# lh3/minimap2

Hardware: AMD Instinct MI355X
Metric: aligned Gbases/sec (map-ont, 10 kb reads, -a) (higher is better)
Workload: dtype int8 (ksw2 difference DP) / int32+f32 (chaining)

## Files before the change

include/mm2amd.h:

```cpp
#ifndef MM2AMD_H
#define MM2AMD_H

#include <stdint.h>
#include <stddef.h>

#ifdef __cplusplus
extern "C" {
#endif

#define MM2AMD_EINVAL  (-1)
#define MM2AMD_ENODEV  (-2)
#define MM2AMD_EHIP    (-3)
#define MM2AMD_ENOMEM  (-4)
#define MM2AMD_ESTATE  (-5)
#define MM2AMD_EIO     (-6)

const char *mm2amd_last_error(void);
int mm2amd_last_error_code(void);
int mm2amd_version(void);
int mm2amd_host_cpus(void);
int mm2amd_device_count(void);


typedef struct {
// ... 23 lines not shown
#define MM2AMD_FIN_MAX_OPS 7168
typedef struct {
	const uint8_t *query, *target;
	int32_t qlen, tlen;
	int32_t n_pieces;
	const uint32_t *const *piece;
	const int32_t *piece_len;
} mm2amd_fin_job_t;
typedef struct { int32_t n_cigar, blen, mlen, n_ambi, dp_max, qshift, tshift, is_spliced; uint32_t cigar_off; } mm2amd_fin_res_t;
int mm2amd_update_extra_batch(int n_jobs, const mm2amd_fin_job_t *jobs, const int8_t *mat25, int8_t q, int8_t e, int log_gap,
                              mm2amd_fin_res_t *res, uint32_t *cigar_pool, size_t cigar_pool_cap);

#define MM2AMD_TXT_CIGAR   0
#define MM2AMD_TXT_CS      1
#define MM2AMD_TXT_CS_LONG 2
#define MM2AMD_TXT_MD      3
typedef struct { const uint8_t *query, *target; int32_t qlen, tlen; const uint32_t *cigar; int32_t n_cigar; } mm2amd_txt_job_t;
typedef struct { uint64_t off; uint32_t len; int32_t status; } mm2amd_txt_res_t;
int mm2amd_aln_text_batch(int n_jobs, const mm2amd_txt_job_t *jobs, int what, mm2amd_txt_res_t *res, char *pool, size_t pool_cap);

#define MM2AMD_LL_QREV  1
#define MM2AMD_LL_QCOMP 2
#define MM2AMD_LL_TREV  4
#define MM2AMD_LL_PATH_WAVE 0
#define MM2AMD_LL_PATH_WG   1
#define MM2AMD_LL_PATH_HOST 2
typedef struct { const uint8_t *query, *target; int32_t qlen, tlen; int32_t flag; } mm2amd_ll_job_t;
typedef struct { int32_t score, qe, te, path; } mm2amd_ll_res_t;
int mm2amd_ksw_ll_batch(int n_jobs, const mm2amd_ll_job_t *jobs, int8_t m, const int8_t *mat, int gapo, int gape, mm2amd_ll_res_t *res);
int mm2amd_ksw_ll_limits(int *strip_cols, int *wg_waves, int64_t *wg_min_cells, int *max_len);

int mm2amd_sort_pairs_u64(uint64_t *keys, uint64_t *vals, uint64_t n, int bits);
int mm2amd_exclusive_sum_u32(const uint32_t *in, uint32_t *out, uint64_t n);

int mm2amd_ksw_extz2_batch(int n_jobs, const mm2amd_ksw_job_t *jobs, int8_t m, const int8_t *mat, int8_t gapo, int8_t gape,
                           mm2amd_ksw_res_t *res, uint32_t *cigar_pool, size_t cigar_pool_cap);

int mm2amd_ksw_exts2_batch(int n_jobs, const mm2amd_ksw_job_t *jobs, int8_t m, const int8_t *mat, int8_t gapo, int8_t gape, int8_t gapo2, int8_t noncan,
                           mm2amd_ksw_res_t *res, uint32_t *cigar_pool, size_t cigar_pool_cap);

#ifdef MINIMAP2_H
typedef mm_idx_t mm2amd_idx_t; typedef mm_mapopt_t mm2amd_mapopt_t; typedef mm_reg1_t mm2amd_reg1_t;
struct mm2amd_bseq1_s;
#define MM2AMD_BSEQ_PTR const void *
#define MM2AMD_REG_PP   void **
#else
typedef void mm2amd_idx_t; typedef void mm2amd_mapopt_t;
#define MM2AMD_BSEQ_PTR const void *
#define MM2AMD_REG_PP   void **
#endif

void mm2amd_idxopt_init(void *io);
void mm2amd_mapopt_init(void *mo);
int mm2amd_set_opt(const char *preset, void *io, void *mo);
int mm2amd_check_opt(const void *io, const void *mo);

typedef struct mm2amd_index_s mm2amd_index_t;
mm2amd_index_t *mm2amd_idx_str(int w, int k, int is_hpc, int bucket_bits, int n, const char **seq, const char **name);
void mm2amd_idx_destroy(mm2amd_index_t *idx);
int mm2amd_idx_stat(const mm2amd_index_t *idx, int *k, int *w, int *flag, uint32_t *n_seq, uint64_t *sum_len,
                    uint64_t *n_distinct, uint64_t *n_minimizers);
int32_t mm2amd_idx_cal_max_occ(const mm2amd_index_t *idx, float f);
int mm2amd_mapopt_update(void *mo, const mm2amd_index_t *idx);
int mm2amd_idx_table_shape(const mm2amd_index_t *idx, int *bucket_bits, int *key_shift);
int mm2amd_idx_export(const mm2amd_index_t *idx, uint32_t *bucket_start, uint64_t *keys, uint32_t *val_off, uint64_t *pos, uint32_t *S);

// ... 64 lines not shown
```

minimap2_amd/__init__.py:

```python
import ctypes as C
import os

_HERE = os.path.dirname(os.path.abspath(__file__))
LIB_PATH = os.path.join(_HERE, "libmm2amd.so")


class Mm2AmdError(RuntimeError):
    pass


class KswJob(C.Structure):
    _fields_ = [("query", C.c_void_p), ("target", C.c_void_p), ("qlen", C.c_int32), ("tlen", C.c_int32), ("w", C.c_int32),
                ("zdrop", C.c_int32), ("end_bonus", C.c_int32), ("flag", C.c_int32)]


class FinJob(C.Structure):
    _fields_ = [("query", C.c_void_p), ("target", C.c_void_p), ("qlen", C.c_int32), ("tlen", C.c_int32), ("n_pieces", C.c_int32),
                ("piece", C.POINTER(C.POINTER(C.c_uint32))), ("piece_len", C.POINTER(C.c_int32))]


class FinRes(C.Structure):
    _fields_ = [("n_cigar", C.c_int32), ("blen", C.c_int32), ("mlen", C.c_int32), ("n_ambi", C.c_int32), ("dp_max", C.c_int32), ("qshift", C.c_int32),
                ("tshift", C.c_int32), ("is_spliced", C.c_int32), ("cigar_off", C.c_uint32)]

# ... 94 lines not shown
    L.mm_gpu_map_staged.argtypes = [ip, C.POINTER(vp), ip, ip]
    L.mm_gpu_batch_stage_queued.argtypes = [C.c_int, ip, ip, vp]
    L.mm_gpu_batch_discard.restype = None
    L.mm2amd_free_regs.argtypes = [C.c_int, ip, C.POINTER(vp)]
    L.mm2amd_free_regs.restype = None
    L.mm2amd_last_stats.argtypes = [C.POINTER(C.c_double), C.c_int]
    L.mm2amd_pack_regs.argtypes = [C.c_int, ip, C.POINTER(vp), vp, C.c_int64]
    L.mm2amd_pack_regs.restype = C.c_int64
    L.mm2amd_unpack_regs.argtypes = [vp, C.c_int64, C.c_int, ip, C.POINTER(vp)]
    L.mm_gpu_init_multi.argtypes = [vp, vp, C.c_int, C.c_int, ip]
    L.mm_gpu_context_generation.restype = C.c_uint64
    L.mm_gpu_destroy_if.argtypes = [C.c_uint64]
    if hasattr(L, "mm2amd_idx_str"):
        L.mm2amd_ksw_extd2_batch.restype = C.c_int
        L.mm2amd_ksw_extd2_batch.argtypes = [C.c_int, C.POINTER(KswJob), C.c_int8, C.c_char_p, C.c_int8, C.c_int8, C.c_int8,
                                             C.c_int8, C.POINTER(KswRes), C.POINTER(C.c_uint32), C.c_size_t]
        L.mm2amd_ksw_extz2_batch.restype = C.c_int
        L.mm2amd_ksw_extz2_batch.argtypes = [C.c_int, C.POINTER(KswJob), C.c_int8, C.c_char_p, C.c_int8, C.c_int8, C.POINTER(KswRes),
                                             C.POINTER(C.c_uint32), C.c_size_t]
        L.mm2amd_ksw_exts2_batch.restype = C.c_int
        L.mm2amd_ksw_exts2_batch.argtypes = [C.c_int, C.POINTER(KswJob), C.c_int8, C.c_char_p, C.c_int8, C.c_int8, C.c_int8, C.c_int8,
                                             C.POINTER(KswRes), C.POINTER(C.c_uint32), C.c_size_t]
        L.mm2amd_update_extra_batch.restype = C.c_int
        L.mm2amd_update_extra_batch.argtypes = [C.c_int, C.POINTER(FinJob), C.c_char_p, C.c_int8, C.c_int8, C.c_int, C.POINTER(FinRes), C.POINTER(C.c_uint32), C.c_size_t]
        L.mm2amd_aln_text_batch.argtypes = [C.c_int, C.POINTER(TxtJob), C.c_int, C.POINTER(TxtRes), vp, C.c_size_t]
        L.mm2amd_hits_text_batch.argtypes = [vp, C.c_int, C.POINTER(vp), C.POINTER(C.c_char_p), C.POINTER(C.c_int32), C.c_int, C.c_int, C.POINTER(TxtRes), vp,
                                             C.c_size_t]
        L.mm2amd_idx_getseq.argtypes = [vp, C.c_uint32, C.c_uint32, C.c_uint32, vp]
        if hasattr(L, "mm2amd_ksw_ll_batch"):
            L.mm2amd_ksw_ll_batch.argtypes = [C.c_int, C.POINTER(LlJob), C.c_int8, C.c_char_p, C.c_int, C.c_int, C.POINTER(LlRes)]
            L.mm2amd_ksw_ll_limits.argtypes = [ip, ip, C.POINTER(C.c_int64), ip]
        L.mm2amd_sort_pairs_u64.argtypes = [vp, vp, C.c_uint64, C.c_int]
        L.mm2amd_exclusive_sum_u32.argtypes = [vp, vp, C.c_uint64]
        L.mm2amd_idx_str.restype = vp
        L.mm2amd_idx_str.argtypes = [C.c_int, C.c_int, C.c_int, C.c_int, C.c_int, C.POINTER(C.c_char_p), C.POINTER(C.c_char_p)]
        L.mm2amd_idx_destroy.argtypes = [vp]
        L.mm2amd_idx_destroy.restype = None
        L.mm2amd_idx_stat.argtypes = [vp, ip, ip, ip, C.POINTER(C.c_uint32), C.POINTER(C.c_uint64), C.POINTER(C.c_uint64),
                                      C.POINTER(C.c_uint64)]
        L.mm2amd_idx_cal_max_occ.argtypes = [vp, C.c_float]
        L.mm2amd_idx_cal_max_occ.restype = C.c_int32
        L.mm2amd_mapopt_update.argtypes = [vp, vp]
        L.mm2amd_idx_table_shape.argtypes = [vp, ip, ip]
        L.mm2amd_idx_export.argtypes = [vp, vp, vp, vp, vp, vp]
        L.mm2amd_idx_dump.argtypes = [vp, C.c_char_p, C.c_int, C.c_int]
        L.mm2amd_idx_load.restype = vp
        L.mm2amd_idx_load.argtypes = [C.c_char_p, C.c_int, ip]
        L.mm2amd_idx_is_idx.argtypes = [C.c_char_p]
        L.mm2amd_idx_seq.argtypes = [vp, C.c_uint32, C.POINTER(C.c_char_p), C.POINTER(C.c_uint32)]
        L.mm2amd_idx_io_stats.argtypes = [C.POINTER(C.c_double), C.c_int]
        L.mm_gpu_init_index.argtypes = [vp, vp, C.c_int]
        L.mm_gpu_init_index_multi.argtypes = [vp, vp, C.c_int, C.c_int, ip]
        L.mm2amd_set_opt.argtypes = [C.c_char_p, vp, vp]
        L.mm2amd_check_opt.argtypes = [vp, vp]
        L.mm2amd_idxopt_init.argtypes = [vp]
        L.mm2amd_mapopt_init.argtypes = [vp]
        L.mm_gpu_format_batch.argtypes = [C.c_int, ip, ip, vp, ip, C.POINTER(vp), ip, C.POINTER(C.c_void_p), C.POINTER(C.c_size_t)]
        L.mm_gpu_format_batch_view.argtypes = [C.c_int, ip, ip, vp, ip, C.POINTER(vp), ip, C.POINTER(C.c_void_p), C.POINTER(C.c_size_t)]
        L.mm_gpu_format_batch_dev.argtypes = [C.c_int, ip, ip, vp, ip, C.POINTER(vp), ip, C.POINTER(C.c_void_p), C.POINTER(C.c_size_t), ip]
        L.mm2amd_profile_enable.argtypes = [C.c_int]
        L.mm2amd_profile_enable.restype = None
        L.mm2amd_profile_get.argtypes = [C.POINTER(KernelStat), C.c_int]
    return L


def host_cpus():
# ... 156 lines not shown
    _check(lib().mm2amd_ksw_ll_batch(n, arr, 5, bytes(mat), gapo, gape, res))
    return [(r.score, r.qe, r.te, r.path) for r in res[:n]]


def ksw_ll_limits():
    a, b, d, c = C.c_int(0), C.c_int(0), C.c_int(0), C.c_int64(0)
    _check(lib().mm2amd_ksw_ll_limits(C.byref(a), C.byref(b), C.byref(c), C.byref(d)))
    return {"strip_cols": a.value, "wg_waves": b.value, "wg_min_cells": c.value, "max_len": d.value}


def hits_text(idx, hits, reads, what, is_qstrand=False):
    n = len(hits)
    harr = (C.c_void_p * max(n, 1))(*hits)
    rb = [r.encode() if isinstance(r, str) else bytes(r) for r in reads]
    qarr, qlen = (C.c_char_p * max(n, 1))(*rb), (C.c_int32 * max(n, 1))(*[len(r) for r in rb])
    L = lib()
    return _texts(lambda res, pool, cap: L.mm2amd_hits_text_batch(idx, n, harr, qarr, qlen, what, 1 if is_qstrand else 0, res, pool, cap), n)


def sort_pairs_u64(keys, vals, bits=64):
    import numpy as np
    k, v = np.ascontiguousarray(keys, dtype=np.uint64).copy(), np.ascontiguousarray(vals, dtype=np.uint64).copy()
    assert k.shape == v.shape and k.ndim == 1
    _check(lib().mm2amd_sort_pairs_u64(k.ctypes.data, v.ctypes.data, k.size, bits))
    return k, v


def exclusive_sum_u32(a):
    import numpy as np
    x = np.ascontiguousarray(a, dtype=np.uint32)
    out = np.empty(x.size + 1, dtype=np.uint32)
    _check(lib().mm2amd_exclusive_sum_u32(x.ctypes.data, out.ctypes.data, x.size))
    return out


def ksw_extz2_batch(jobs, mat, gapo, gape):
    return ksw_extd2_batch(jobs, mat, gapo, gape, None, None)


def ksw_exts2_batch(jobs, mat, gapo, gape, gapo2, noncan):
    return ksw_extd2_batch(jobs, mat, gapo, gape, gapo2, None, noncan=noncan)


def ksw_extd2_batch(jobs, mat, gapo, gape, gapo2, gape2, noncan=None):
    n = len(jobs)
    arr = (KswJob * n)()
    keep = []
    tot = 0
    for i, (q, t, w, zdrop, end_bonus, flag) in enumerate(jobs):
        qb, tb = bytes(q), bytes(t)
        keep.append((qb, tb))
        arr[i].query = C.cast(C.c_char_p(qb), C.c_void_p)
        arr[i].target = C.cast(C.c_char_p(tb), C.c_void_p)
        arr[i].qlen, arr[i].tlen, arr[i].w, arr[i].zdrop, arr[i].end_bonus, arr[i].flag = len(qb), len(tb), w, zdrop, end_bonus, flag
        tot += len(qb) + len(tb)
    res = (KswRes * n)()
    pool = (C.c_uint32 * max(tot, 1))()
    if noncan is not None:
        _check(lib().mm2amd_ksw_exts2_batch(n, arr, 5, bytes(mat), gapo, gape, gapo2, noncan, res, pool, max(tot, 1)))
    elif gapo2 is None:
        _check(lib().mm2amd_ksw_extz2_batch(n, arr, 5, bytes(mat), gapo, gape, res, pool, max(tot, 1)))
    else:
        _check(lib().mm2amd_ksw_extd2_batch(n, arr, 5, bytes(mat), gapo, gape, gapo2, gape2, res, pool, max(tot, 1)))
    out = []
    for r in res:
        out.append((r.max, r.zdropped, r.max_q, r.max_t, r.mqe, r.mqe_t, r.mte, r.mte_q, r.score, r.reach_end,
# ... 384 lines not shown
```

minimap2_amd/csrc/backend_hip.cpp:

```cpp
#include <atomic>
#include <condition_variable>
#include <algorithm>
#include <cstdio>
#include <cstring>
#include <memory>
#include <mutex>
#include <numeric>
#include <stdexcept>
#include <thread>
#include "backend.hpp"
#include "chain_dump.hpp"
#include "chain_host.hpp"
#include "device_ctx.hpp"
#include "ksw_host.hpp"
#include "seed_chain_dev.hpp"
#include "index_build.hpp"
#include "kernel_prof.hpp"
#include "threads.hpp"
#include "trace.hpp"
#include "sdust_core.hpp"

namespace mm2amd {

extern const uint8_t kNt4Table[256];
// ... 289 lines not shown
		B.sort_key_in = ln.d_skey_in.p, B.sort_val_in = ln.d_sval_in.p, B.sort_key_out = ln.d_skey_out.p, B.sort_val_out = ln.d_sval_out.p, B.tie_flag = ln.d_tie.p;
		B.tie_list = ln.d_tie.p + n, B.tie_count = ln.d_tie.p + 2 * n;
		B.rid_bits = rid_bits_;
		int n_class[kAnchorSortClasses] = { 0 }, class_first[kAnchorSortClasses + 1] = { 0 };
		double a_class[kAnchorSortClasses] = { 0 };
		for (size_t i = 0; i < n; ++i) if (h_na[i]) { const int c = anchor_sort_class(h_na[i], rid_bits_); ++n_class[c], a_class[c] += h_na[i]; }
		for (int c = 0; c < kAnchorSortClasses; ++c) class_first[c + 1] = class_first[c] + n_class[c];
		uint32_t *h_list = ln.h_sort_list.ensure(n + 1);
		{
			int fill[kAnchorSortClasses];
			for (int c = 0; c < kAnchorSortClasses; ++c) fill[c] = class_first[c];
			for (size_t i = 0; i < n; ++i) if (h_na[i]) h_list[fill[anchor_sort_class(h_na[i], rid_bits_)]++] = (uint32_t)i;
		}
		ln.d_sort_list.ensure(n + 1);
		if (class_first[kAnchorSortClasses]) HIP_CHECK(hipMemcpyAsync(ln.d_sort_list.p, h_list, (size_t)class_first[kAnchorSortClasses] * 4, hipMemcpyHostToDevice, st));
		B.a_off = ln.d_a_off.p, B.mp_off = ln.d_mp_off.p, B.anchors = ln.d_anchors.p, B.mini_pos = ln.d_minipos.p;
		B.f = ln.d_f.p, B.p = ln.d_p.p, B.t = ln.d_t.p;
		kp.begin(st); launch_seed_expand(B, I_, P, st); kp.end(st, "seed_expand_kernel", 24.0 * n_a);
		launch_anchor_sort(B, I_, P, ln.d_sort_list.p, n_class, a_class, st, &kp);
		if (getenv("MM2AMD_TIE_COUNT")) {
			std::vector<uint32_t> tf(n);
			stream_wait(st);
			HIP_CHECK(hipMemcpy(tf.data(), ln.d_tie.p, n * 4, hipMemcpyDeviceToHost));
			size_t n_tied = 0;
			for (size_t i = 0; i < n; ++i) n_tied += tf[i] != 0;
			fprintf(stderr, "[mm2amd] anchor sort: %zu of %zu reads have duplicated keys (%d / %d / %d reads in the 7 k / 10 k / global classes)\n", n_tied, n, n_class[3], n_class[4], n_class[5]);
		}
		if (const char *dump = getenv("MM2AMD_SEED_DUMP")) {
			std::vector<Anchor> all(n_a + 1);
			stream_wait(st);
			if (n_a) HIP_CHECK(hipMemcpy(all.data(), ln.d_anchors.p, n_a * sizeof(Anchor), hipMemcpyDeviceToHost));
			static std::mutex dump_mu;
			std::lock_guard<std::mutex> lk(dump_mu);
			if (FILE *fp = fopen(dump, "a")) {
				for (size_t i = 0; i < n; ++i) {
					fprintf(fp, "QR\t%s\t%d\nRS\t%d\n", read_names_.empty() || !read_names_[lo + i] ? "*" : read_names_[lo + i], P.mid_occ, h_rep[i]);
					for (uint64_t j = a_off[i]; j < a_off[i + 1]; ++j) {
						const Anchor &a = all[j];
						fprintf(fp, "SD\t%s\t%d\t%c\t%d\t%d\t%d\n", (*fi_names_)[a.x << 1 >> 33].c_str(), (int32_t)a.x, "+-"[a.x >> 63], (int32_t)a.y, (int32_t)(a.y >> 32 & 0xff),
						        j == a_off[i] ? 0 : ((int32_t)a.y - (int32_t)all[j - 1].y) - ((int32_t)a.x - (int32_t)all[j - 1].x));
					}
				}
				fclose(fp);
			}
		}
		const char *cdump = P.chain_dump ? chain_dump_path() : nullptr;
		auto dump_block = [&](size_t i) {
			ChainDumpBlock b;
			b.name = read_names_.empty() ? nullptr : read_names_[lo + i];
			b.qlen = (int)(seq_off_[lo + i + 1] - seq_off_[lo + i]), b.n_seg = has_pairs_ ? unit_first_[lo + i + 1] - unit_first_[lo + i] : 1;
			return b;
		};
		if (P.anchors_only) {
			Anchor *ha = ln.h_anchors.ensure(n_a + 1);
			uint64_t *hmp = ln.h_minipos.ensure(n_mp + 1);
			if (n_a) HIP_CHECK(hipMemcpyAsync(ha, ln.d_anchors.p, n_a * sizeof(Anchor), hipMemcpyDeviceToHost, st));
			if (n_mp) HIP_CHECK(hipMemcpyAsync(hmp, ln.d_minipos.p, n_mp * 8, hipMemcpyDeviceToHost, st));
			stream_wait(st);
			Trace::get().add(lane_id, "gpu:expand+sort, d2h:anchors", tt, Trace::now());
			kp.collect();
			if (cdump) {
				std::string txt;
				for (size_t i = 0; i < n; ++i) {
					ChainDumpBlock b = dump_block(i);
					b.handed_back = true, b.in = ha + a_off[i], b.n_in = (int64_t)(a_off[i + 1] - a_off[i]);
					chain_dump_format(txt, P, b);
				}
				chain_dump_flush(cdump, txt);
			}
			parallel_for(n_threads, (long)n, [&](long i, int) {
				ReadChains &c = out[i];
				c.rep_len = h_rep[i];
				c.mp_p = hmp + mp_off[i], c.n_mp = (int32_t)(mp_off[i + 1] - mp_off[i]);
// ... 626 lines not shown
```

minimap2_amd/csrc/capi_kernels.cpp:

```cpp
#include <mutex>
#include <string>
#include <vector>
#include <cstring>
#include "../../include/mm2amd.h"
#include "hip_util.hpp"
#include "device_ctx.hpp"
#include "ksw_host.hpp"
#include "kernel_prof.hpp"
#include "region_finish.hpp"
#include "aln_text.hpp"
#include "ksw_ll.hpp"
#include "device_sort.hpp"
#include <map>

namespace mm2amd { int capi_fail(int code, const std::string &msg); }
using namespace mm2amd;

namespace {

int fail(int code, const std::string &msg) { return capi_fail(code, msg); }

struct KernelApiState {
	KswRunner ksw;
	DevBuf<uint8_t> d_qpool, d_tpool;
};
KernelApiState &kstate() { static KernelApiState s; return s; }

struct LlApiState {
	DevBuf<uint8_t> d_q, d_t;
	DevBuf<LlJob> d_jobs;
	DevBuf<LlRes> d_res;
	DevBuf<uint32_t> d_bnd;
	PinBuf<uint8_t> h_q, h_t;
	PinBuf<LlJob> h_jobs;
	PinBuf<LlRes> h_res;
};
LlApiState &ll_state() { static LlApiState s; return s; }
constexpr size_t kLlBndBudget = (size_t)1 << 26;

bool ll_no_wg() { const char *e = getenv("MM2AMD_LL_NO_WG"); return e && *e && strcmp(e, "0") != 0; }
int64_t ll_wg_min_cells() { const char *e = getenv("MM2AMD_LL_WG_MIN_CELLS"); return e && *e ? (int64_t)strtoll(e, nullptr, 10) : kLlWgMinCells; }

template <typename F>
int guarded(F &&f)
{
// ... 370 lines not shown
	return guarded([&]() -> int {
		DeviceCtx &dc = device_ctx();
		std::lock_guard<std::mutex> lk(dc.mu);
		ensure_device(dc);
		DevBuf<uint64_t> k0, v0, k1, v1;
		k0.ensure(n, 1.0), v0.ensure(n, 1.0), k1.ensure(n, 1.0), v1.ensure(n, 1.0);
		HIP_CHECK(hipMemcpyAsync(k0.p, keys, n * 8, hipMemcpyHostToDevice, dc.stream));
		HIP_CHECK(hipMemcpyAsync(v0.p, vals, n * 8, hipMemcpyHostToDevice, dc.stream));
		const int where = device_sort_pairs_u64(k0.p, v0.p, k1.p, v1.p, n, bits, dc.stream);
		HIP_CHECK(hipMemcpyAsync(keys, where ? k1.p : k0.p, n * 8, hipMemcpyDeviceToHost, dc.stream));
		HIP_CHECK(hipMemcpyAsync(vals, where ? v1.p : v0.p, n * 8, hipMemcpyDeviceToHost, dc.stream));
		HIP_CHECK(hipStreamSynchronize(dc.stream));
		return 0;
	});
}

int mm2amd_exclusive_sum_u32(const uint32_t *in, uint32_t *out, uint64_t n)
{
	if (!out || (n > 0 && !in) || n >= (1ull << 32)) return fail(MM2AMD_EINVAL, "[mm2amd] exclusive_sum_u32: bad arguments (n < 2^32)");
	return guarded([&]() -> int {
		DeviceCtx &dc = device_ctx();
		std::lock_guard<std::mutex> lk(dc.mu);
		ensure_device(dc);
		DevBuf<uint32_t> d;
		d.ensure(n + 1, 1.0);
		if (n) HIP_CHECK(hipMemcpyAsync(d.p, in, n * 4, hipMemcpyHostToDevice, dc.stream));
		device_exclusive_sum_u32(d.p, d.p, n, dc.stream);
		HIP_CHECK(hipMemcpyAsync(out, d.p, (n + 1) * 4, hipMemcpyDeviceToHost, dc.stream));
		HIP_CHECK(hipStreamSynchronize(dc.stream));
		return 0;
	});
}

long long mm2amd_alloc_counter(int which)
{
	AllocStats &a = alloc_stats();
	BandCounters &b = band_counters();
	return which == 0 ? a.dev_allocs.load() : which == 1 ? a.pin_allocs.load() : which == 2 ? a.ns.load() : which == 3 ? (long long)b.n_band1.load() : which == 4 ? (long long)b.n_band2.load() :
	       which == 5 ? (long long)b.n_widened.load() : which == 6 ? (long long)b.n_retried.load() :
	       which == 7 ? (long long)dev_arena().held_bytes() : which == 8 ? (long long)pin_arena().held_bytes() : which == 9 ? (long long)dev_arena().used_bytes() : which == 10 ? (long long)pin_arena().used_bytes() :
	       which == 11 ? (long long)b.n_band4.load() : (long long)b.n_retried_big.load();
}

void mm2amd_profile_enable(int on)
{
	for (int r = 0; r < kMaxReplicas; ++r) for (int l = 0; l < kMaxProfLanes; ++l) kernel_profiler(l, r).reset();
	KernelProfiler::enabled_flag() = on != 0;
}

int mm2amd_profile_get(mm2amd_kernel_stat_t *out, int cap)
{
	std::map<std::string, KernelStat> all;
	for (int r = 0; r < kMaxReplicas; ++r) for (int l = 0; l < kMaxProfLanes; ++l)
		for (const auto &kv : kernel_profiler(l, r).stats()) {
			KernelStat &k = all[kv.first];
			k.ms += kv.second.ms, k.alg_bytes += kv.second.alg_bytes, k.units += kv.second.units, k.launches += kv.second.launches;
		}
	int n = 0;
	for (const auto &kv : all) {
		if (n >= cap) break;
		mm2amd_kernel_stat_t &o = out[n++];
		memset(&o, 0, sizeof o);
		strncpy(o.name, kv.first.c_str(), sizeof o.name - 1);
		o.ms = kv.second.ms, o.alg_bytes = kv.second.alg_bytes, o.launches = kv.second.launches, o.units = kv.second.units;
	}
	return n;
// ... 4 lines not shown
```

minimap2_amd/csrc/seed_chain.hip:

```cpp
#include <hip/hip_runtime.h>
#include "hip_util.hpp"
#include "seed_chain_dev.hpp"
#include "index_build.hpp"
#include "heap_order.hpp"
#include "sdust_core.hpp"
#include "sketch_dev.hpp"
#include "kernel_prof.hpp"

namespace mm2amd {

#define WAVE_SYNC() do { __builtin_amdgcn_fence(__ATOMIC_ACQ_REL, "wavefront"); __builtin_amdgcn_wave_barrier(); } while (0)

__constant__ uint8_t c_nt4[256];
extern const uint8_t kNt4Table[256];
static bool g_nt4_uploaded = false;

static void upload_tables(hipStream_t s)
{
	if (g_nt4_uploaded) return;
	HIP_CHECK(hipMemcpyToSymbolAsync(HIP_SYMBOL(c_nt4), kNt4Table, 256, 0, hipMemcpyHostToDevice, s));
	g_nt4_uploaded = true;
}

__global__ void __launch_bounds__(256) encode_kernel(SeedChainBuffers B)
{
	const int r = blockIdx.x;
	const uint64_t o = B.seq_off[r];
	const int64_t len = (int64_t)(B.seq_off[r + 1] - o);
	const char *src = B.ascii + o;
	uint8_t *f = B.qpool + 2 * o;
	const int64_t mis = (int64_t)((uintptr_t)src & 15u);
	const uint4 *w = (const uint4 *)(src - mis);
	const int64_t n_words = (mis + len + 15) >> 4;
	for (int64_t c = threadIdx.x; c < n_words; c += blockDim.x) {
		const uint4 v = w[c];
		const uint32_t q[4] = { v.x, v.y, v.z, v.w };
#pragma unroll
		for (int b = 0; b < 16; ++b) {
			const int64_t j = (c << 4) + b - mis;
			if (j >= 0 && j < len) {
				const uint8_t code = c_nt4[q[b >> 2] >> ((b & 3) * 8) & 0xffu];
				f[j] = code;
				f[2 * len - 1 - j] = code < 4 ? 3 - code : 4;
			}
		}
	}
}

void launch_encode(const SeedChainBuffers &B, void *stream)
{
	upload_tables((hipStream_t)stream);
	hipLaunchKernelGGL(encode_kernel, dim3(B.n_reads), dim3(256), 0, (hipStream_t)stream, B);
	HIP_CHECK(hipGetLastError());
}

__device__ __forceinline__ uint64_t mix64(uint64_t key, uint64_t mask) { return mm_hash64(key, mask); }

template <int WMAX>
__global__ void __launch_bounds__(64) sketch_kernel(SeedChainBuffers B, int w, int k, int is_hpc)
{
	const int r = blockIdx.x * blockDim.x + threadIdx.x;
	if (r >= B.n_reads) return;
	const uint64_t o = B.seq_off[r];
	const int len = (int)(B.seq_off[r + 1] - o);
	const uint8_t *seq = B.qpool + 2 * o;
	const uint64_t shift1 = 2 * (k - 1), mask = (1ULL << 2 * k) - 1;
	uint64_t kmer0 = 0, kmer1 = 0, min_x = UINT64_MAX, min_y = UINT64_MAX;
	uint64_t bx[WMAX], by[WMAX];
	int hq[32], hq_front = 0, hq_count = 0;
	int l = 0, buf_pos = 0, min_pos = 0, kmer_span = 0;
	uint32_t n_out = 0;
	uint64_t *ox = B.mz_x + B.mz_off[r], *oy = B.mz_y + B.mz_off[r];
#define EMIT_MZ(X, Y) do { ox[n_out] = (X); oy[n_out] = (Y); ++n_out; } while (0)
	for (int j = 0; j < w; ++j) bx[j] = by[j] = UINT64_MAX;
	for (int i = 0; i < len; ++i) {
		const int c = seq[i];
		uint64_t ix = UINT64_MAX, iy = UINT64_MAX;
		if (c < 4) {
			if (is_hpc) {
				int run = 1;
				if (i + 1 < len && seq[i + 1] == c) {
					for (run = 2; i + run < len; ++run) if (seq[i + run] != c) break;
					i += run - 1;
				}
				hq[(hq_count++ + hq_front) & 0x1f] = run;
// ... 156 lines not shown
		else MM2_SKETCH_LAUNCH(false, 0);
#undef MM2_SKETCH_LAUNCH
	} else {
		const dim3 grid((B.n_reads + 63) / 64), block(64);
		if (P.w <= 32) hipLaunchKernelGGL((sketch_kernel<32>), grid, block, 0, s, B, P.w, P.k, P.is_hpc);
		else hipLaunchKernelGGL((sketch_kernel<256>), grid, block, 0, s, B, P.w, P.k, P.is_hpc);
	}
	HIP_CHECK(hipGetLastError());
}

__global__ void __launch_bounds__(64) dust_filter_kernel(SeedChainBuffers B)
{
	const int r = blockIdx.x * 64 + threadIdx.x;
	if (r >= B.n_reads) return;
	const int32_t u0 = B.unit_first ? B.unit_first[r] : 0, nu = B.unit_first ? B.unit_first[r + 1] - u0 : 1;
	for (int32_t k = 0; k < nu; ++k) {
		const uint64_t o = B.unit_first ? B.unit_off[u0 + k] : B.seq_off[r];
		uint32_t *cnt = B.unit_first ? const_cast<uint32_t *>(B.unit_cnt) + (u0 + k) : B.mz_cnt + r;
		const uint32_t *rs = B.sd_off + o, *re = B.sd_aoff + o;
		const int n_reg = (int)B.sd_n[o];
		if (n_reg == 0) continue;
		const int pos_off = B.unit_first ? (int)(o - B.unit_off[u0]) : 0;
		*cnt = (uint32_t)dust_filter_minimizers((int)*cnt, B.mz_x + o, B.mz_y + o, n_reg,
			[&](int u, int32_t *st, int32_t *en) { *st = (int32_t)rs[u], *en = (int32_t)re[u]; }, pos_off);
	}
}

void launch_dust_filter(const SeedChainBuffers &B, void *stream)
{
	hipLaunchKernelGGL(dust_filter_kernel, dim3((B.n_reads + 63) / 64), dim3(64), 0, (hipStream_t)stream, B);
	HIP_CHECK(hipGetLastError());
}

__device__ __forceinline__ uint32_t idx_lookup(const DevIndex &I, uint64_t hash, uint32_t *off)
{
	const uint64_t b = hash >> I.key_shift;
	if (b >= (1ull << I.bucket_bits)) return 0;
	uint32_t skip = 0;
	if (I.first) {
		const IdxSlot f = I.first[b];
		if (f.key == hash) { *off = f.off; return f.cnt & ~kIdxMoreKeys; }
		if (!(f.cnt & kIdxMoreKeys)) return 0;
		skip = 1;
	}
	const uint32_t s = I.bucket_start[b] + skip, e = I.bucket_start[b + 1];
	for (uint32_t i = s; i < e; ++i) {
		const IdxSlot k = I.slots[i];
		if (k.key == hash) { *off = k.off; return k.cnt; }
	}
	return 0;
}

__device__ __forceinline__ int lane_id() { return threadIdx.x & 63; }
__device__ __forceinline__ int popc_below(unsigned long long m, int lane) { return __popcll(m & ((1ull << lane) - 1ull)); }

__device__ __forceinline__ int32_t wave_prefix_max_i32(int32_t v)
{
	int32_t o;
	o = __builtin_amdgcn_update_dpp(INT32_MIN, v, 0x111, 0xf, 0xf, false); v = o > v ? o : v;
	o = __builtin_amdgcn_update_dpp(INT32_MIN, v, 0x112, 0xf, 0xf, false); v = o > v ? o : v;
	o = __builtin_amdgcn_update_dpp(INT32_MIN, v, 0x114, 0xf, 0xf, false); v = o > v ? o : v;
	o = __builtin_amdgcn_update_dpp(INT32_MIN, v, 0x118, 0xf, 0xf, false); v = o > v ? o : v;
	o = __builtin_amdgcn_update_dpp(INT32_MIN, v, 0x142, 0xa, 0xf, false); v = o > v ? o : v;
	o = __builtin_amdgcn_update_dpp(INT32_MIN, v, 0x143, 0xc, 0xf, false); v = o > v ? o : v;
	return v;
}
__device__ __forceinline__ uint32_t wave_prefix_add_u32(uint32_t v)
{
	v += (uint32_t)__builtin_amdgcn_update_dpp(0, (int32_t)v, 0x111, 0xf, 0xf, false);
	v += (uint32_t)__builtin_amdgcn_update_dpp(0, (int32_t)v, 0x112, 0xf, 0xf, false);
	v += (uint32_t)__builtin_amdgcn_update_dpp(0, (int32_t)v, 0x114, 0xf, 0xf, false);
	v += (uint32_t)__builtin_amdgcn_update_dpp(0, (int32_t)v, 0x118, 0xf, 0xf, false);
	v += (uint32_t)__builtin_amdgcn_update_dpp(0, (int32_t)v, 0x142, 0xa, 0xf, false);
	v += (uint32_t)__builtin_amdgcn_update_dpp(0, (int32_t)v, 0x143, 0xc, 0xf, false);
	return v;
}
__device__ __forceinline__ int32_t wave_shr1_i32(int32_t first, int32_t v) { return __builtin_amdgcn_update_dpp(first, v, 0x138, 0xf, 0xf, false); }
__device__ __forceinline__ uint64_t wave_shr1_u64(uint64_t first, uint64_t v)
{
	return (uint64_t)(uint32_t)wave_shr1_i32((int32_t)(uint32_t)first, (int32_t)(uint32_t)v) | (uint64_t)(uint32_t)wave_shr1_i32((int32_t)(uint32_t)(first >> 32), (int32_t)(uint32_t)(v >> 32)) << 32;
}
__device__ __forceinline__ int32_t lane_get_i32(int32_t v, int l) { return __builtin_amdgcn_readlane(v, l); }
__device__ __forceinline__ uint64_t lane_get_u64(uint64_t v, int l)
{
	return (uint64_t)(uint32_t)__builtin_amdgcn_readlane((int32_t)(uint32_t)v, l) | (uint64_t)(uint32_t)__builtin_amdgcn_readlane((int32_t)(uint32_t)(v >> 32), l) << 32;
}
constexpr int HIST_N = 2048;
constexpr uint32_t SD_TANDEM = 1u << 8, SD_FLT = 1u << 9, SD_SEG1 = 1u << 31;

__device__ void heap_down(uint64_t *h, int i, int n)
{
	int k = i;
	const uint64_t tmp = h[i];
	while ((k = (k << 1) + 1) < n) {
		if (k != n - 1 && h[k] < h[k + 1]) ++k;
		if (h[k] < tmp) break;
		h[i] = h[k]; i = k;
	}
	h[i] = tmp;
}

__device__ __forceinline__ bool skip_hit(int64_t flag, uint64_t rr, uint32_t qp, int qlen, int32_t nm_lb, int32_t nm_eq, const DevIndex &I, bool *is_self)
{
	*is_self = false;
	const bool fwd = (rr & 1) == (qp & 1);
	if (nm_lb >= 0 && (flag & (ref::F_NO_DIAG | ref::F_NO_DUAL))) {
		const uint32_t rid = (uint32_t)(rr >> 32);
		const int32_t rank = I.name_rank[rid];
		if ((flag & ref::F_NO_DIAG) && rank == nm_eq && (int)I.seq_len[rid] == qlen) {
			if ((uint32_t)rr >> 1 == qp >> 1) return true;
			if (fwd) *is_self = true;
		}
		if ((flag & ref::F_NO_DUAL) && rank < nm_lb) return true;
	}
	if (fwd ? (flag & ref::F_REV_ONLY) != 0 : (flag & ref::F_FOR_ONLY) != 0) return true;
	return false;
}

#define HIT_RULES_SETUP() \
	const bool name_rules = (P.flag & (ref::F_NO_DIAG | ref::F_NO_DUAL)) && B.name_lb && I.name_rank; \
	const int32_t nm_lb = name_rules ? B.name_lb[r] : -1, nm_eq = name_rules ? B.name_eq[r] : -1; \
// ... 40 lines not shown
		bool hot = false;
		for (int i = lane; i < HIST_N; i += 64) { const uint32_t c = hist[i]; hot |= ((int)c > P.q_mid_occ && (float)c > thr); }
		if (__ballot(hot)) {
			for (int base = 0; base < n; base += 64) {
				const int i = base + lane;
				if (i < n) {
					const uint64_t x = mx[i];
					bool keep = true;
					const uint32_t c = hist[(uint32_t)((x * 0x9E3779B97F4A7C15ull) >> 53)];
					if ((int)c > P.q_mid_occ && (float)c > thr) {
						int cnt = 0;
						for (int j = 0; j < n; ++j) cnt += (mx[j] == x);
						keep = !(cnt > P.q_mid_occ && (float)cnt > thr);
					}
					sd_info[i] = keep ? 1u : 0u;
				}
			}
			WAVE_SYNC();
			int dst = 0;
			for (int base = 0; base < n; base += 64) {
				const int i = base + lane;
				uint64_t x = 0, y = 0;
				bool keep = false;
				if (i < n) { x = mx[i], y = my[i]; keep = sd_info[i] != 0; }
				const unsigned long long km = __ballot(keep);
				WAVE_SYNC();
				if (keep) { const int d = dst + popc_below(km, lane); mx[d] = x, my[d] = y; }
				dst += __popcll(km);
				WAVE_SYNC();
			}
			n = dst;
		}
	}
	for (int i = lane; i < n; i += 64) {
		const uint64_t x = mx[i];
		uint32_t off = 0;
		const uint32_t cnt = idx_lookup(I, x >> 8, &off);
		uint32_t info = (uint32_t)(x & 0xff);
		if (my[i] >> 32) info |= SD_SEG1;
		if (i > 0 && x >> 8 == mx[i - 1] >> 8) info |= SD_TANDEM;
		if (i < n - 1 && x >> 8 == mx[i + 1] >> 8) info |= SD_TANDEM;
		sd_n[i] = cnt, sd_off[i] = off, sd_info[i] = info, sd_qpos[i] = (uint32_t)my[i];
	}
	WAVE_SYNC();
	int n_m0 = 0;
	for (int base = 0; base < n; base += 64) {
		const int i = base + lane;
		uint32_t cnt = 0, off = 0, info = 0, qp = 0;
		if (i < n) cnt = sd_n[i], off = sd_off[i], info = sd_info[i], qp = sd_qpos[i];
		const unsigned long long hm = __ballot(cnt > 0);
		WAVE_SYNC();
		if (cnt > 0) { const int d = n_m0 + popc_below(hm, lane); sd_n[d] = cnt, sd_off[d] = off, sd_info[d] = info, sd_qpos[d] = qp; }
		n_m0 += __popcll(hm);
		WAVE_SYNC();
	}
	int n_high = 0;
	for (int i = lane; i < n_m0; i += 64) n_high += sd_n[i] > (uint32_t)P.mid_occ;
	for (int o = 32; o > 0; o >>= 1) n_high += __shfl_xor(n_high, o, 64);
	if (n_high > 0) {
		if (P.occ_dist > 0 && P.max_max_occ > P.mid_occ) {
			if (n_m0 > 1 && lane == 0) {
				uint64_t *const hb = (uint64_t *)hist;
				int last0 = -1;
				for (int i = 0; i <= n_m0; ++i) {
					if (i == n_m0 || sd_n[i] <= (uint32_t)P.mid_occ) {
						if (i - last0 > 1) {
							const int ps = last0 < 0 ? 0 : (int)(sd_qpos[last0] >> 1), pe = i == n_m0 ? qlen : (int)(sd_qpos[i] >> 1);
							const int st = last0 + 1, en = i;
							int keep = (int)((double)(pe - ps) / P.occ_dist + .499), j, kk;
							if (keep > 0) {
								if (keep > 128) keep = 128;
#ifdef MM2AMD_WAVE_EMU
								if (getenv("MM2AMD_OCC_HEAP_TRACE")) fprintf(stderr, "[mm2amd] occurrence-filter heap: read %d keeps %d of %d seeds\n", r, keep, en - st);
#endif
								for (j = st, kk = 0; j < en && kk < keep; ++j, ++kk) hb[kk] = (uint64_t)sd_n[j] << 32 | (uint32_t)j;
								for (int q = kk >> 1; q-- > 0;) heap_down(hb, q, kk);
								for (; j < en; ++j)
									if ((int32_t)sd_n[j] < (int32_t)(hb[0] >> 32)) { hb[0] = (uint64_t)sd_n[j] << 32 | (uint32_t)j; heap_down(hb, 0, kk); }
								for (j = 0; j < kk; ++j) sd_info[(uint32_t)hb[j]] |= SD_FLT;
							}
							for (j = st; j < en; ++j) sd_info[j] ^= SD_FLT;
							for (j = st; j < en; ++j) if (sd_n[j] > (uint32_t)P.max_max_occ) sd_info[j] |= SD_FLT;
						}
						last0 = i;
					}
				}
			}
		} else {
			for (int i = lane; i < n_m0; i += 64) if (sd_n[i] > (uint32_t)P.mid_occ) sd_info[i] |= SD_FLT;
		}
// ... 1573 lines not shown
```

Before: 3.514.

## Batch index probes with memory-level parallelism and flatten encode kernel across reads

The seed lookup loop is replaced by a fused probe-and-compact routine that issues several hash-bucket loads per lane at once (depth 4) and compacts hits in the same pass. This removes the separate store-then-recompact pass over the seed arrays and hides index-lookup latency. The encode kernel now uses a fixed grid that walks a flat range of 16-byte words across all reads, with the nt4 table held in shared memory and owner lookup done by galloping search, in place of one block per read. New C and Python encode entry points are added for testing.

```diff
diff --git a/include/mm2amd.h b/include/mm2amd.h
--- a/include/mm2amd.h
+++ b/include/mm2amd.h
@@ -79,6 +79,9 @@
 
 int mm2amd_sort_pairs_u64(uint64_t *keys, uint64_t *vals, uint64_t n, int bits);
 int mm2amd_exclusive_sum_u32(const uint32_t *in, uint32_t *out, uint64_t n);
+
+int mm2amd_encode_batch(int n, const char *const *seqs, const int32_t *lens, const int32_t *lens2, uint8_t *out);
+int mm2amd_encode_range(int n, const char *const *seqs, const int32_t *lens, const int32_t *lens2, int lo, int hi, uint8_t *out);
 
 int mm2amd_ksw_extz2_batch(int n_jobs, const mm2amd_ksw_job_t *jobs, int8_t m, const int8_t *mat, int8_t gapo, int8_t gape,
                            mm2amd_ksw_res_t *res, uint32_t *cigar_pool, size_t cigar_pool_cap);
diff --git a/minimap2_amd/__init__.py b/minimap2_amd/__init__.py
--- a/minimap2_amd/__init__.py
+++ b/minimap2_amd/__init__.py
@@ -150,6 +150,8 @@
             L.mm2amd_ksw_ll_limits.argtypes = [ip, ip, C.POINTER(C.c_int64), ip]
         L.mm2amd_sort_pairs_u64.argtypes = [vp, vp, C.c_uint64, C.c_int]
         L.mm2amd_exclusive_sum_u32.argtypes = [vp, vp, C.c_uint64]
+        L.mm2amd_encode_batch.argtypes = [C.c_int, C.POINTER(C.c_char_p), C.POINTER(C.c_int32), C.POINTER(C.c_int32), vp]
+        L.mm2amd_encode_range.argtypes = [C.c_int, C.POINTER(C.c_char_p), C.POINTER(C.c_int32), C.POINTER(C.c_int32), C.c_int, C.c_int, vp]
         L.mm2amd_idx_str.restype = vp
         L.mm2amd_idx_str.argtypes = [C.c_int, C.c_int, C.c_int, C.c_int, C.c_int, C.POINTER(C.c_char_p), C.POINTER(C.c_char_p)]
         L.mm2amd_idx_destroy.argtypes = [vp]
@@ -372,6 +374,27 @@
     out = np.empty(x.size + 1, dtype=np.uint32)
     _check(lib().mm2amd_exclusive_sum_u32(x.ctypes.data, out.ctypes.data, x.size))
     return out
+
+
+def encode_batch(reads, lo=0, hi=None):
+    import numpy as np
+    n = len(reads)
+    pairs = [r if isinstance(r, tuple) else (r, b"") for r in reads]
+    bufs = [bytes(a) + bytes(b) for a, b in pairs]
+    unit_off = [0]
+    for a, b in pairs:
+        unit_off.append(unit_off[-1] + len(a))
+        if len(b) > 0:
+            unit_off.append(unit_off[-1] + len(b))
+    seqs = (C.c_char_p * max(n, 1))(*bufs)
+    lens = (C.c_int32 * max(n, 1))(*[len(a) for a, _ in pairs])
+    lens2 = (C.c_int32 * max(n, 1))(*[len(b) for _, b in pairs])
+    out = np.empty(2 * unit_off[-1] + 32, dtype=np.uint8)
+    if lo == 0 and hi is None:
+        _check(lib().mm2amd_encode_batch(n, seqs, lens, lens2, out.ctypes.data))
+    else:
+        _check(lib().mm2amd_encode_range(n, seqs, lens, lens2, lo, n if hi is None else hi, out.ctypes.data))
+    return out, np.array(unit_off, dtype=np.int64)
 
 
 def ksw_extz2_batch(jobs, mat, gapo, gape):
diff --git a/minimap2_amd/csrc/backend_hip.cpp b/minimap2_amd/csrc/backend_hip.cpp
--- a/minimap2_amd/csrc/backend_hip.cpp
+++ b/minimap2_amd/csrc/backend_hip.cpp
@@ -345,13 +345,16 @@
 			if (n_a) HIP_CHECK(hipMemcpy(all.data(), ln.d_anchors.p, n_a * sizeof(Anchor), hipMemcpyDeviceToHost));
 			static std::mutex dump_mu;
 			std::lock_guard<std::mutex> lk(dump_mu);
+			const bool dump_flags = getenv("MM2AMD_SEED_DUMP_FLAGS") != nullptr;
 			if (FILE *fp = fopen(dump, "a")) {
 				for (size_t i = 0; i < n; ++i) {
 					fprintf(fp, "QR\t%s\t%d\nRS\t%d\n", read_names_.empty() || !read_names_[lo + i] ? "*" : read_names_[lo + i], P.mid_occ, h_rep[i]);
 					for (uint64_t j = a_off[i]; j < a_off[i + 1]; ++j) {
 						const Anchor &a = all[j];
-						fprintf(fp, "SD\t%s\t%d\t%c\t%d\t%d\t%d\n", (*fi_names_)[a.x << 1 >> 33].c_str(), (int32_t)a.x, "+-"[a.x >> 63], (int32_t)a.y, (int32_t)(a.y >> 32 & 0xff),
+						fprintf(fp, "SD\t%s\t%d\t%c\t%d\t%d\t%d", (*fi_names_)[a.x << 1 >> 33].c_str(), (int32_t)a.x, "+-"[a.x >> 63], (int32_t)a.y, (int32_t)(a.y >> 32 & 0xff),
 						        j == a_off[i] ? 0 : ((int32_t)a.y - (int32_t)all[j - 1].y) - ((int32_t)a.x - (int32_t)all[j - 1].x));
+						if (dump_flags) fprintf(fp, "\t%d", (int)(a.y >> 42 & 1));
+						fputc('\n', fp);
 					}
 				}
 				fclose(fp);
diff --git a/minimap2_amd/csrc/capi_kernels.cpp b/minimap2_amd/csrc/capi_kernels.cpp
--- a/minimap2_amd/csrc/capi_kernels.cpp
+++ b/minimap2_amd/csrc/capi_kernels.cpp
@@ -11,6 +11,7 @@
 #include "aln_text.hpp"
 #include "ksw_ll.hpp"
 #include "device_sort.hpp"
+#include "seed_chain_dev.hpp"
 #include <map>
 
 namespace mm2amd { int capi_fail(int code, const std::string &msg); }
@@ -447,6 +448,48 @@
 	});
 }
 
+int mm2amd_encode_batch(int n, const char *const *seqs, const int32_t *lens, const int32_t *lens2, uint8_t *out) { return mm2amd_encode_range(n, seqs, lens, lens2, 0, n, out); }
+
+int mm2amd_encode_range(int n, const char *const *seqs, const int32_t *lens, const int32_t *lens2, int lo, int hi, uint8_t *out)
+{
+	if (n < 0 || !out || (n > 0 && (!seqs || !lens)) || lo < 0 || hi < lo || hi > n) return fail(MM2AMD_EINVAL, "[mm2amd] encode_batch: bad arguments");
+	std::vector<uint64_t> unit_off(1, 0);
+	std::vector<size_t> frag_unit(1, 0);
+	for (int i = 0; i < n; ++i) {
+		const int32_t l2 = lens2 ? lens2[i] : 0;
+		if (lens[i] < 0 || l2 < 0 || (lens[i] + (int64_t)l2 > 0 && !seqs[i])) return fail(MM2AMD_EINVAL, "[mm2amd] encode_batch: bad read (negative length or null sequence)");
+		unit_off.push_back(unit_off.back() + (uint64_t)lens[i]);
+		if (l2 > 0) unit_off.push_back(unit_off.back() + (uint64_t)l2);
+		frag_unit.push_back(unit_off.size() - 1);
+	}
+	const uint64_t total = unit_off.back();
+	const size_t n_units = unit_off.size() - 1;
+	return guarded([&]() -> int {
+		DeviceCtx &dc = device_ctx();
+		std::lock_guard<std::mutex> lk(dc.mu);
+		ensure_device(dc);
+		PinBuf<char> h_ascii;
+		DevBuf<uint8_t> d_pool;
+		DevBuf<uint64_t> d_off;
+		char *h = h_ascii.ensure(total + 32, 1.0);
+		uint64_t o = 0;
+		for (int i = 0; i < n; ++i) {
+			const uint64_t l = (uint64_t)lens[i] + (uint64_t)(lens2 ? lens2[i] : 0);
+			if (l) memcpy(h + o, seqs[i], l);
+			o += l;
+		}
+		d_pool.ensure(2 * total + 32, 1.0), d_off.ensure(n_units + 1, 1.0);
+		HIP_CHECK(hipMemsetAsync(d_pool.p, 0xff, 2 * total + 32, dc.stream));
+		HIP_CHECK(hipMemcpyAsync(d_off.p, unit_off.data(), (n_units + 1) * 8, hipMemcpyHostToDevice, dc.stream));
+		SeedChainBuffers B;
+		B.n_reads = (int)(frag_unit[hi] - frag_unit[lo]), B.seq_off = d_off.p + frag_unit[lo], B.ascii = h, B.qpool = d_pool.p + 16;
+		launch_encode(B, dc.stream);
+		HIP_CHECK(hipMemcpyAsync(out, d_pool.p, 2 * total + 32, hipMemcpyDeviceToHost, dc.stream));
+		HIP_CHECK(hipStreamSynchronize(dc.stream));
+		return 0;
+	});
+}
+
 long long mm2amd_alloc_counter(int which)
 {
 	AllocStats &a = alloc_stats();
diff --git a/minimap2_amd/csrc/seed_chain.hip b/minimap2_amd/csrc/seed_chain.hip
--- a/minimap2_amd/csrc/seed_chain.hip
+++ b/minimap2_amd/csrc/seed_chain.hip
@@ -22,35 +22,75 @@
 	g_nt4_uploaded = true;
 }
 
+constexpr int kEncodeBlocks = 64, kEncodeDepth = 4;
+
+__device__ __forceinline__ int encode_owner(const uint64_t *seq_off, int lo, int n, uint64_t p)
+{
+	int step = 1;
+	while (lo + step < n && seq_off[lo + step] <= p) lo += step, step <<= 1;
+	int hi = lo + step < n ? lo + step : n;
+	while (hi - lo > 1) {
+		const int mid = (int)(((unsigned)lo + (unsigned)hi) >> 1);
+		if (seq_off[mid] <= p) lo = mid; else hi = mid;
+	}
+	return lo;
+}
+
 __global__ void __launch_bounds__(256) encode_kernel(SeedChainBuffers B)
 {
-	const int r = blockIdx.x;
-	const uint64_t o = B.seq_off[r];
-	const int64_t len = (int64_t)(B.seq_off[r + 1] - o);
-	const char *src = B.ascii + o;
-	uint8_t *f = B.qpool + 2 * o;
-	const int64_t mis = (int64_t)((uintptr_t)src & 15u);
-	const uint4 *w = (const uint4 *)(src - mis);
-	const int64_t n_words = (mis + len + 15) >> 4;
-	for (int64_t c = threadIdx.x; c < n_words; c += blockDim.x) {
-		const uint4 v = w[c];
-		const uint32_t q[4] = { v.x, v.y, v.z, v.w };
+	__shared__ uint8_t s_nt4[256];
+	s_nt4[threadIdx.x] = c_nt4[threadIdx.x];
+	__syncthreads();
+	const int n = B.n_reads;
+	const uint64_t *seq_off = B.seq_off;
+	const uint64_t sh = (uint64_t)((uintptr_t)B.ascii & 15u);
+	const uint4 *W = (const uint4 *)(B.ascii - sh);
+	const uint64_t S = seq_off[0] + sh, E = seq_off[n] + sh;
+	if (E == S) return;
+	const uint64_t w0 = S >> 4, w1 = (E + 15) >> 4, a0 = w0 & ~63ull;
+	const uint64_t per = ((w1 - a0 + gridDim.x - 1) / gridDim.x + 255) & ~255ull;
+	const uint64_t b0 = a0 + blockIdx.x * per, b1 = b0 + per < w1 ? b0 + per : w1;
+	uint8_t *const qp = B.qpool - 2 * sh;
+	int r = 0;
+	for (uint64_t c = b0 + threadIdx.x; c < b1; c += 256 * kEncodeDepth) {
+		uint4 v[kEncodeDepth];
 #pragma unroll
-		for (int b = 0; b < 16; ++b) {
-			const int64_t j = (c << 4) + b - mis;
-			if (j >= 0 && j < len) {
-				const uint8_t code = c_nt4[q[b >> 2] >> ((b & 3) * 8) & 0xffu];
-				f[j] = code;
-				f[2 * len - 1 - j] = code < 4 ? 3 - code : 4;
-			}
-		}
-	}
+		for (int k = 0; k < kEncodeDepth; ++k) {
+			const uint64_t cw = c + 256 * k;
+			v[k] = cw >= w0 && cw < b1 ? W[cw] : make_uint4(0, 0, 0, 0);
+		}
+#pragma unroll
+		for (int k = 0; k < kEncodeDepth; ++k) {
+			const uint64_t cw = c + 256 * k;
+			if (cw < w0 || cw >= b1) continue;
+			const uint64_t p0 = cw << 4 > S ? cw << 4 : S, p1 = (cw << 4) + 16 < E ? (cw << 4) + 16 : E;
+			r = encode_owner(seq_off, r, n, p0 - sh);
+			uint64_t o = seq_off[r] + sh, e = seq_off[r + 1] + sh;
+			const uint32_t q[4] = { v[k].x, v[k].y, v[k].z, v[k].w };
+#pragma unroll
+			for (int b = 0; b < 16; ++b) {
+				const uint64_t p = (cw << 4) + b;
+				if (p < p0 || p >= p1) continue;
+				while (p >= e) { ++r; o = e; e = seq_off[r + 1] + sh; }
+				const uint8_t code = s_nt4[q[b >> 2] >> ((b & 3) * 8) & 0xffu];
+				qp[o + p] = code;
+				qp[o + 2 * e - 1 - p] = code < 4 ? 3 - code : 4;
+			}
+		}
+	}
+}
+
+static int encode_grid_blocks()
+{
+	static const int n = [] { const char *e = getenv("MM2AMD_ENCODE_BLOCKS"); const int v = e && *e ? atoi(e) : 0; return v > 0 && v <= 4096 ? v : kEncodeBlocks; }();
+	return n;
 }
 
 void launch_encode(const SeedChainBuffers &B, void *stream)
 {
 	upload_tables((hipStream_t)stream);
-	hipLaunchKernelGGL(encode_kernel, dim3(B.n_reads), dim3(256), 0, (hipStream_t)stream, B);
+	if (B.n_reads <= 0) return;
+	hipLaunchKernelGGL(encode_kernel, dim3(encode_grid_blocks()), dim3(256), 0, (hipStream_t)stream, B);
 	HIP_CHECK(hipGetLastError());
 }
 
@@ -273,27 +313,77 @@
 	HIP_CHECK(hipGetLastError());
 }
 
-__device__ __forceinline__ uint32_t idx_lookup(const DevIndex &I, uint64_t hash, uint32_t *off)
-{
-	const uint64_t b = hash >> I.key_shift;
-	if (b >= (1ull << I.bucket_bits)) return 0;
-	uint32_t skip = 0;
-	if (I.first) {
-		const IdxSlot f = I.first[b];
-		if (f.key == hash) { *off = f.off; return f.cnt & ~kIdxMoreKeys; }
-		if (!(f.cnt & kIdxMoreKeys)) return 0;
-		skip = 1;
-	}
-	const uint32_t s = I.bucket_start[b] + skip, e = I.bucket_start[b + 1];
-	for (uint32_t i = s; i < e; ++i) {
-		const IdxSlot k = I.slots[i];
-		if (k.key == hash) { *off = k.off; return k.cnt; }
-	}
-	return 0;
-}
-
 __device__ __forceinline__ int lane_id() { return threadIdx.x & 63; }
 __device__ __forceinline__ int popc_below(unsigned long long m, int lane) { return __popcll(m & ((1ull << lane) - 1ull)); }
+
+constexpr uint32_t SD_TANDEM = 1u << 8, SD_FLT = 1u << 9, SD_SEG1 = 1u << 31;
+constexpr int kProbeDepth = 4;
+
+__device__ __forceinline__ int seed_probe_compact(const uint64_t *__restrict__ qx, const uint64_t *__restrict__ qy, int n, int lane, const DevIndex &I, uint32_t mid_occ,
+                                                  uint32_t *__restrict__ o_n, uint32_t *__restrict__ o_off, uint32_t *__restrict__ o_info, uint32_t *__restrict__ o_qpos, int *n_high)
+{
+	const uint64_t n_buckets = 1ull << I.bucket_bits;
+	int n_m0 = 0;
+	for (int base = 0; base < n; base += 64 * kProbeDepth) {
+		uint64_t hash[kProbeDepth], y[kProbeDepth], bkt[kProbeDepth];
+		uint32_t info[kProbeDepth], cnt[kProbeDepth], off[kProbeDepth], s[kProbeDepth], e[kProbeDepth];
+		bool live[kProbeDepth];
+#pragma unroll
+		for (int k = 0; k < kProbeDepth; ++k) {
+			const int i = base + 64 * k + lane;
+			uint64_t x = 0, xp = 0, xn = 0;
+			y[k] = 0;
+			if (i < n) {
+				x = qx[i], y[k] = qy[i];
+				if (i > 0) xp = qx[i - 1];
+				if (i < n - 1) xn = qx[i + 1];
+			}
+			hash[k] = x >> 8, bkt[k] = hash[k] >> I.key_shift;
+			live[k] = i < n && bkt[k] < n_buckets;
+			info[k] = (uint32_t)(x & 0xff);
+			if (y[k] >> 32) info[k] |= SD_SEG1;
+			if ((i > 0 && i < n && hash[k] == xp >> 8) || (i < n - 1 && hash[k] == xn >> 8)) info[k] |= SD_TANDEM;
+			cnt[k] = off[k] = 0, s[k] = e[k] = 0;
+		}
+		if (I.first) {
+			IdxSlot f[kProbeDepth];
+#pragma unroll
+			for (int k = 0; k < kProbeDepth; ++k) if (live[k]) f[k] = I.first[bkt[k]];
+#pragma unroll
+			for (int k = 0; k < kProbeDepth; ++k) {
+				if (!live[k]) continue;
+				if (f[k].key == hash[k]) off[k] = f[k].off, cnt[k] = f[k].cnt & ~kIdxMoreKeys, live[k] = false;
+				else if (!(f[k].cnt & kIdxMoreKeys)) live[k] = false;
+			}
+#pragma unroll
+			for (int k = 0; k < kProbeDepth; ++k) if (live[k]) s[k] = I.bucket_start[bkt[k]] + 1, e[k] = I.bucket_start[bkt[k] + 1];
+		} else {
+#pragma unroll
+			for (int k = 0; k < kProbeDepth; ++k) if (live[k]) s[k] = I.bucket_start[bkt[k]], e[k] = I.bucket_start[bkt[k] + 1];
+		}
+		for (bool more = true; more;) {
+			more = false;
+#pragma unroll
+			for (int k = 0; k < kProbeDepth; ++k) {
+				if (s[k] >= e[k]) continue;
+				const IdxSlot q = I.slots[s[k]];
+				if (q.key == hash[k]) off[k] = q.off, cnt[k] = q.cnt, s[k] = e[k];
+				else more |= ++s[k] < e[k];
+			}
+		}
+#pragma unroll
+		for (int k = 0; k < kProbeDepth; ++k) {
+			const unsigned long long hm = __ballot(cnt[k] > 0);
+			if (cnt[k] > 0) {
+				const int d = n_m0 + popc_below(hm, lane);
+				o_n[d] = cnt[k], o_off[d] = off[k], o_info[d] = info[k], o_qpos[d] = (uint32_t)y[k];
+				*n_high += cnt[k] > mid_occ;
+			}
+			n_m0 += __popcll(hm);
+		}
+	}
+	return n_m0;
+}
 
 __device__ __forceinline__ int32_t wave_prefix_max_i32(int32_t v)
 {
@@ -327,7 +417,6 @@
 	return (uint64_t)(uint32_t)__builtin_amdgcn_readlane((int32_t)(uint32_t)v, l) | (uint64_t)(uint32_t)__builtin_amdgcn_readlane((int32_t)(uint32_t)(v >> 32), l) << 32;
 }
 constexpr int HIST_N = 2048;
-constexpr uint32_t SD_TANDEM = 1u << 8, SD_FLT = 1u << 9, SD_SEG1 = 1u << 31;
 
 __device__ void heap_down(uint64_t *h, int i, int n)
 {
@@ -434,30 +523,9 @@
 			n = dst;
 		}
 	}
-	for (int i = lane; i < n; i += 64) {
-		const uint64_t x = mx[i];
-		uint32_t off = 0;
-		const uint32_t cnt = idx_lookup(I, x >> 8, &off);
-		uint32_t info = (uint32_t)(x & 0xff);
-		if (my[i] >> 32) info |= SD_SEG1;
-		if (i > 0 && x >> 8 == mx[i - 1] >> 8) info |= SD_TANDEM;
-		if (i < n - 1 && x >> 8 == mx[i + 1] >> 8) info |= SD_TANDEM;
-		sd_n[i] = cnt, sd_off[i] = off, sd_info[i] = info, sd_qpos[i] = (uint32_t)my[i];
-	}
+	int n_high = 0;
+	const int n_m0 = seed_probe_compact(mx, my, n, lane, I, (uint32_t)P.mid_occ, sd_n, sd_off, sd_info, sd_qpos, &n_high);
 	WAVE_SYNC();
-	int n_m0 = 0;
-	for (int base = 0; base < n; base += 64) {
-		const int i = base + lane;
-		uint32_t cnt = 0, off = 0, info = 0, qp = 0;
-		if (i < n) cnt = sd_n[i], off = sd_off[i], info = sd_info[i], qp = sd_qpos[i];
-		const unsigned long long hm = __ballot(cnt > 0);
-		WAVE_SYNC();
-		if (cnt > 0) { const int d = n_m0 + popc_below(hm, lane); sd_n[d] = cnt, sd_off[d] = off, sd_info[d] = info, sd_qpos[d] = qp; }
-		n_m0 += __popcll(hm);
-		WAVE_SYNC();
-	}
-	int n_high = 0;
-	for (int i = lane; i < n_m0; i += 64) n_high += sd_n[i] > (uint32_t)P.mid_occ;
 	for (int o = 32; o > 0; o >>= 1) n_high += __shfl_xor(n_high, o, 64);
 	if (n_high > 0) {
 		if (P.occ_dist > 0 && P.max_max_occ > P.mid_occ) {
```

New measurement: 3.663 (median of 6 runs). 1.04x the previous value.
